# DmSM-1/C-OFDM

Hardware: AMD Instinct MI355X
Metric: IQ-samples/sec (tx IFFT+CP and rx FFT+equalise), 2048-subcarrier frames, 1/2/4/8 GPU (higher is better)
Workload: dtype f64

## Files before the change

### c-ofdm_amd/csrc/ofdm_capi.cpp

```cpp
#include <dlfcn.h>
#include <hip/hip_runtime.h>

#include <algorithm>
#include <climits>
#include <cctype>
#include <cmath>
#include <complex>
#include <cstdarg>
#include <cstdio>
#include <cstdlib>
#include <chrono>
#include <mutex>
#include <cstring>
#include <fstream>
#include <iterator>
#include <random>
#include <stdexcept>
#include <string>
#include <unordered_map>
#include <vector>

#include "../../include/ofdm_mi355x.h"

#if __has_include(<rccl/rccl.h>)
// ... 66 lines not shown
            return fail(OFDM_ERR_PARSE, "stol failed for key '%s': %s", key.c_str(), e.what());
        }
    }
    return OFDM_OK;
}

template <class T>
int upload(T** dst, const std::vector<T>& v)
{
    HIP_TRY(hipMalloc((void**)dst, std::max<size_t>(1, v.size()) * sizeof(T)));
    if (!v.empty()) HIP_TRY(hipMemcpy(*dst, v.data(), v.size() * sizeof(T), hipMemcpyHostToDevice));
    return OFDM_OK;
}

}

struct ofdm_ctx {
    ofdm_params p{};
    int device = 0;
    int logn = 0;
    int N = 0, D = 0, P = 0, cp = 0, S = 0, k = 0, L = 0, seg = 0, npr = 0, t2 = 0;
    ofdm_geometry geo{};
    std::vector<cd> t2_symbol, ofdm_preamble, mod_preamble, templ;
    std::vector<uint8_t> preamble_bytes;
    std::vector<double> t2_mask;
    double2* d_tw = nullptr;
    int* d_data_bin = nullptr;
    int* d_data_slot = nullptr;
    int* d_pilot_bin = nullptr;
    int* d_bin_map = nullptr;
    int* d_rx_pack = nullptr;
    int* d_pilot_swz = nullptr;
    int* d_tx_code = nullptr;
    double2* d_const = nullptr;
    double2* d_const_bpsk = nullptr;
    double dec_tau[3] = {};
    bool dec_fast = false;
    double2* d_header = nullptr;
    double2* d_preamble = nullptr;
    double2* d_templ = nullptr;
    double2* d_tspec = nullptr;
    float2* d_tspec32 = nullptr;
    double2* d_twm = nullptr;
    double tspec_max = 0.0;
    double2* d_modpre = nullptr;
    double* d_t2mask = nullptr;
    double2* d_t2tw = nullptr;
    int* d_first = nullptr;
    int t2_logn = -1;
    struct CfoPlan {
        int nsym = 0, logm = -1, g = 0;
        double2* tw_sub = nullptr;
        double2* tw_full = nullptr;
        int* borders = nullptr;
    };
    std::vector<CfoPlan> cfo_plans;
    double* d_cfo_scratch = nullptr;
    size_t cfo_scratch_n = 0;
    double2* d_scratch = nullptr;
    size_t scratch_bytes = 0;
    struct Grow {
        void* p = nullptr;
        size_t bytes = 0;
    };
    Grow s_walk, s_batch, s_chan, s_pbs;
    static constexpr size_t PRE_SCRATCH_STARTS = 64;
// ... 127 lines not shown
    {
        std::vector<char> used(N, 0);
        const long step = D / P + 1, seg = D / P, half = P / 2;
        long j = 0;
        auto take = [&](long b) {
            if (b < 1 || b >= N || used[b]) return false;
            used[b] = 1;
            return true;
        };
        for (long pos = 1 + seg; j < half; ++j, pos += step) {
            if (!take(pos)) return fail(OFDM_ERR_INVALID, "pilot comb does not fit fft_size");
            for (long t = 0; t < seg; ++t)
                if (!take(pos - seg + t)) return fail(OFDM_ERR_INVALID, "data segments do not fit fft_size");
        }
        for (long pos = N - step * half; j < P; ++j, pos += step) {
            if (!take(pos)) return fail(OFDM_ERR_INVALID, "pilot comb does not fit fft_size");
            for (long t = 0; t < seg; ++t)
                if (!take(pos + 1 + t)) return fail(OFDM_ERR_INVALID, "data segments do not fit fft_size");
        }
    }
    if (p->t2sin_size < 0 || (p->t2sin_size && (p->t2_sin_f1 < 0 || p->t2_sin_f1 >= p->t2sin_size ||
                                                p->t2_sin_f2 < 0 || p->t2_sin_f2 >= p->t2sin_size)))
        return fail(OFDM_ERR_INVALID, "T2 tones outside T2sin_size");
    if (p->pr_sin_len < 0 || p->pr_sin_len > (N + p->cp_size) * p->num_pr_symb)
        return fail(OFDM_ERR_INVALID, "pr_sin_len exceeds the preamble");
    return OFDM_OK;
}

int ofdm_destroy(ofdm_ctx* c)
{
    if (!c) return OFDM_OK;
    (void)hipSetDevice(c->device);
    void* ptrs[] = {c->d_tw, c->d_data_bin, c->d_data_slot, c->d_pilot_bin, c->d_bin_map, c->d_rx_pack,
                    c->d_pilot_swz, c->d_tx_code, c->d_const,
                    c->d_const_bpsk, c->d_header, c->d_preamble, c->d_templ, c->d_tspec, c->d_tspec32, c->d_twm, c->d_modpre,
                    c->d_t2mask,
                    c->d_t2tw, c->d_first, c->d_scratch, c->d_cfo_scratch, c->d_pre_hv, c->d_pre_done};
    for (void* q : ptrs)
        if (q) (void)hipFree(q);
    for (auto* g : {&c->s_walk, &c->s_batch, &c->s_chan, &c->s_pbs, &c->s_pub, &c->s_chain})
        if (g->p) (void)hipFree(g->p);
    for (auto* g : {&c->h_walk, &c->h_frames, &c->h_status})
        if (g->p) (void)hipHostFree(g->p);
    if (c->d_queue) (void)hipFree(c->d_queue);
    if (c->d_rxq) (void)hipFree(c->d_rxq);
    if (c->ev_call) (void)hipEventDestroy(c->ev_call);
    if (c->ev_walk) (void)hipEventDestroy(c->ev_walk);
    if (c->ev_wdone) (void)hipEventDestroy(c->ev_wdone);
    if (c->side) (void)hipStreamDestroy(c->side);
    for (hipEvent_t ev : c->ev_phase)
        if (ev) (void)hipEventDestroy(ev);
    for (auto& pl : c->cfo_plans) {
        if (pl.tw_sub) (void)hipFree(pl.tw_sub);
        if (pl.tw_full) (void)hipFree(pl.tw_full);
        if (pl.borders) (void)hipFree(pl.borders);
    }
    delete c;
    return OFDM_OK;
}

using ofdm::twiddles;

static std::vector<double2> constellation(int k)
{
    std::vector<double2> t(1u << k);
    if (k == 1) {
        const double step = M_PI * 2 / (double)2;
// ... 50 lines not shown

    std::vector<int> pilot(c->P), segst(c->P), data_bin(c->D), data_slot(c->D), bin_map(c->N, -1);
    {
        const int step = c->seg + 1, half = c->P / 2;
        int j = 0;
        for (int pos = 1 + c->seg; j < half; ++j, pos += step) {
            pilot[j] = pos;
            segst[j] = pos - c->seg;
        }
        for (int pos = c->N - step * half; j < c->P; ++j, pos += step) {
            pilot[j] = pos;
            segst[j] = pos + 1;
        }
        for (int jj = 0; jj < c->P; ++jj) {
            g.pilot_bin[jj] = pilot[jj];
            g.segment_bin[jj] = segst[jj];
            bin_map[pilot[jj]] = -2;
            for (int t = 0; t < c->seg; ++t) {
                const int d = jj * c->seg + t;
                data_bin[d] = segst[jj] + t;
                data_slot[d] = jj;
                bin_map[segst[jj] + t] = d;
            }
        }
    }
    std::vector<int> rx_pack(std::max(c->D, ofdm::RX_DPT * (c->N / 8)), 0),
        pilot_swz(std::max(c->P, c->N / 8), 0);
    for (int d = 0; d < c->D; ++d) rx_pack[d] = ofdm::lds_swz_host(data_bin[d]) | (data_slot[d] << 16);
    for (int j = 0; j < c->P; ++j) pilot_swz[j] = ofdm::lds_swz_host(pilot[j]);
    std::vector<int> tx_code(c->N);
    for (int b = 0; b < c->N; ++b)
        tx_code[b] = bin_map[b] >= 0 ? ofdm::tx_code_data(bin_map[b])
                                     : ofdm::tx_code_fixed(bin_map[b] == -2 ? ofdm::TX_LDS_PILOT : ofdm::TX_LDS_ZERO);
    if ((rc = upload(&c->d_rx_pack, rx_pack)) || (rc = upload(&c->d_pilot_swz, pilot_swz)) ||
        (rc = upload(&c->d_tx_code, tx_code)) ||
        (rc = upload(&c->d_tw, twiddles(c->N))) || (rc = upload(&c->d_data_bin, data_bin)) ||
        (rc = upload(&c->d_data_slot, data_slot)) || (rc = upload(&c->d_pilot_bin, pilot)) ||
        (rc = upload(&c->d_bin_map, bin_map)) || (rc = upload(&c->d_const, constellation(c->k))) ||
        (rc = upload(&c->d_const_bpsk, constellation(1)))) {
        ofdm_destroy(c);
        return rc;
    }

    if (c->k == 2) {
        double* d_tau = nullptr;
        double h_tau[4] = {};
        hipError_t e = hipMalloc((void**)&d_tau, sizeof(h_tau));
        if (e == hipSuccess) e = ofdm::launch_decide_tau_scan(c->k, d_tau, nullptr);
        if (e == hipSuccess) e = hipMemcpy(h_tau, d_tau, sizeof(h_tau), hipMemcpyDeviceToHost);
        if (d_tau) (void)hipFree(d_tau);
        if (e != hipSuccess) {
            ofdm_destroy(c);
            return hip_fail(e, "decision threshold scan");
        }
        for (int j = 0; j < 3; ++j) c->dec_tau[j] = h_tau[j];
        c->dec_fast = h_tau[3] == 1.0;
    }

    c->t2_symbol.assign(c->t2, cd(0, 0));
    if (c->t2) {
        std::vector<cd> spec(c->t2, cd(0, 0));
        spec[params->t2_sin_f1] = cd(0.5, 0);
        spec[params->t2_sin_f2] = cd(0.5, 0);
        for (int n = 0; n < c->t2; ++n) {
            cd acc(0, 0);
            for (int kk = 0; kk < c->t2; ++kk) {
// ... 201 lines not shown
    } else {
        return fail(OFDM_ERR_UNSUPPORTED, "pilot_freq_sinh: form length %ld is not 2^a or 5*2^a (64 <= 2^a <= %d)", S,
                    4096);
    }
    const int P = c->P;
    const double rel_bw = double(c->D + c->P) / (c->N);
    const double rel_pilot_w = rel_bw / P;
    const int pilot_w = int(S * rel_pilot_w);
    std::vector<int> borders(P + 2);
    for (int i = 0, j = int((1.0 - rel_bw - rel_pilot_w) / 2.0 * S); i < P + 2; i++) {
        borders[i] = j;
        j += pilot_w;
    }
    borders[0] = std::max(0, borders[0]);
    for (int b : borders)
        if (b < 0 || b > S) return fail(OFDM_ERR_UNSUPPORTED, "pilot_freq_sinh windows leave the spectrum");
    int rc;
    if ((rc = upload(&pl.tw_sub, twiddles(1 << pl.logm))) || (rc = upload(&pl.borders, borders))) return rc;
    if (pl.g == 5 && (rc = upload(&pl.tw_full, twiddles((int)S)))) return rc;
    c->cfo_plans.push_back(pl);
    *out = &c->cfo_plans.back();
    return OFDM_OK;
}

int ofdm_get_geometry(const ofdm_ctx* c, ofdm_geometry* o)
{
    if (!c || !o) return fail(OFDM_ERR_INVALID, "null argument");
    *o = c->geo;
    return OFDM_OK;
}

int ofdm_rx_emit_fast(const ofdm_ctx* c) { return c ? (c->dec_fast ? 1 : 0) : -1; }

int ofdm_get_t2_symbol(const ofdm_ctx* c, double* o)
{
    if (!c || !o) return fail(OFDM_ERR_INVALID, "null argument");
    std::memcpy(o, c->t2_symbol.data(), c->t2_symbol.size() * sizeof(cd));
    return OFDM_OK;
}

int ofdm_get_preamble(const ofdm_ctx* c, uint8_t* bytes, double* pre, double* modp, double* templ)
{
    if (!c) return fail(OFDM_ERR_INVALID, "null ctx");
    if (bytes) std::memcpy(bytes, c->preamble_bytes.data(), c->preamble_bytes.size());
    if (pre) std::memcpy(pre, c->ofdm_preamble.data(), c->ofdm_preamble.size() * sizeof(cd));
    if (modp) std::memcpy(modp, c->mod_preamble.data(), c->mod_preamble.size() * sizeof(cd));
    if (templ) std::memcpy(templ, c->templ.data(), c->templ.size() * sizeof(cd));
    return OFDM_OK;
}

int ofdm_device_alloc(ofdm_ctx* c, size_t bytes, void** d)
{
    if (!c || !d) return fail(OFDM_ERR_INVALID, "null argument");
    HIP_TRY(hipSetDevice(c->device));
    HIP_TRY(hipMalloc(d, std::max<size_t>(bytes, 1)));
    return OFDM_OK;
}
int ofdm_device_free(ofdm_ctx* c, void* d)
{
    if (!c) return fail(OFDM_ERR_INVALID, "null ctx");
    if (d) HIP_TRY(hipFree(d));
    return OFDM_OK;
}
int ofdm_memcpy_h2d(ofdm_ctx* c, void* dst, const void* src, size_t n, void* st)
{
    if (!c) return fail(OFDM_ERR_INVALID, "null ctx");
// ... 94 lines not shown
    return OFDM_OK;
}

static bool aligned16(const void* p) { return ((uintptr_t)p & 15) == 0; }

static int grow(ofdm_ctx* c, ofdm_ctx::Grow& g, size_t need)
{
    if (need <= g.bytes) return OFDM_OK;
    HIP_TRY(hipSetDevice(c->device));
    if (g.p) HIP_TRY(hipFree(g.p));
    g.p = nullptr;
    g.bytes = 0;
    HIP_TRY(hipMalloc(&g.p, need));
    g.bytes = need;
    return OFDM_OK;
}

static int grow_host(ofdm_ctx* c, ofdm_ctx::Grow& g, size_t need)
{
    if (need <= g.bytes) return OFDM_OK;
    HIP_TRY(hipSetDevice(c->device));
    if (g.p) HIP_TRY(hipHostFree(g.p));
    g.p = nullptr;
    g.bytes = 0;
    HIP_TRY(hipHostMalloc(&g.p, need, hipHostMallocDefault));
    g.bytes = need;
    return OFDM_OK;
}

static void fill_tx(const ofdm_ctx* c, ofdm::TxArgs& a, const uint8_t* bytes, size_t nframes, double* iq,
                    size_t stride, int16_t* iq16, const ofdm_channel* ch)
{
    a.tab = c->tables(false);
    a.bytes = bytes;
    a.iq = reinterpret_cast<double2*>(iq);
    a.iq16 = iq16;
    a.nframes = (long)nframes;
    a.frame_stride = (long)stride;
    a.S = c->S;
    a.D = c->D;
    a.P = c->P;
    a.cp = c->cp;
    a.k = c->k;
    a.bytes_per_frame = c->geo.bytes_per_frame;
    a.pilot_ampl = (double)c->p.pilot_ampl / 1000;
    a.inv_sqrt_n = 1.0 / std::sqrt((double)c->N);
    a.mult = (double)c->p.mult;
    if (ch && ch->noise_std > 0.0) {
        a.noise_scale = ch->noise_std * M_SQRT1_2;
        a.seed = ch->seed;
        a.sample_offset = ch->sample_offset;
    }
}

int ofdm_tx_modulate(ofdm_ctx* c, const uint8_t* bytes, size_t nframes, double* iq_out, size_t frame_stride,
                     int16_t* iq16_out, const ofdm_channel* ch, void* stream)
{
    if (!c || !bytes || !iq_out) return fail(OFDM_ERR_INVALID, "null argument");
    if (frame_stride < (size_t)c->geo.message_len) return fail(OFDM_ERR_INVALID, "frame_stride < message_len");
    if (!aligned16(iq_out)) return fail(OFDM_ERR_INVALID, "iq_out must be 16-byte aligned");
    if (nframes == 0) return OFDM_OK;
    if (nframes * (size_t)c->S > 0x7fffffffu) return fail(OFDM_ERR_INVALID, "too many symbols in one call");
    ofdm::TxArgs a{};
    fill_tx(c, a, bytes, nframes, iq_out, frame_stride, iq16_out, ch);
    hipError_t e = ofdm::launch_tx(c->logn, a, (hipStream_t)stream);
    if (e != hipSuccess) return hip_fail(e, "tx_kernel launch");
// ... 1511 lines not shown
```

### c-ofdm_amd/csrc/ofdm_fft.hpp

```cpp
#pragma once
#include <hip/hip_runtime.h>
#include <cfloat>

#ifdef OFDM_PHASE_MARKS
#define OFDM_PHASE(name) asm volatile("; OFDM_PHASE " #name)
#else
#define OFDM_PHASE(name) ((void)0)
#endif

namespace ofdm {

static __device__ int g_decode_stop = 1 << 30;
#define OFDM_STOP(PROF, k)                                                   \
    do {                                                                     \
        if constexpr (PROF) {                                                \
            if ((k) >= g_decode_stop) __builtin_amdgcn_endpgm();             \
        }                                                                    \
    } while (0)

__device__ __forceinline__ double2 cadd(double2 a, double2 b) { return make_double2(a.x + b.x, a.y + b.y); }
__device__ __forceinline__ double2 csub(double2 a, double2 b) { return make_double2(a.x - b.x, a.y - b.y); }

__device__ __forceinline__ double2 cmul(double2 a, double2 b)
{
// ... 143 lines not shown
{
    lds_tw[p.dst] = p.w;
}

template <int LOGN, int JMAX = (1 << LOGN)>
__device__ __forceinline__ double2 tw_get(const double2* __restrict__ lds_tw, int j)
{
    constexpr int NHI = TwLds<LOGN>::NHI;
    const int lo = j & 63;
    const double2 wlo = lds_tw[NHI + (lo ^ ((lo >> 4) & 3))];
    if constexpr (NHI == 1 || JMAX <= 64) return wlo;
    return cmul(lds_tw[j >> 6], wlo);
}

template <int SIGN>
__device__ __forceinline__ void dft2(double2& a, double2& b)
{
    const double2 t = a;
    a = cadd(t, b);
    b = csub(t, b);
}

template <int SIGN>
__device__ __forceinline__ void dft4(double2& a0, double2& a1, double2& a2, double2& a3)
{
    const double2 t0 = cadd(a0, a2), t1 = csub(a0, a2);
    const double2 t2 = cadd(a1, a3), t3 = mul_j<SIGN>(csub(a1, a3));
    a0 = cadd(t0, t2);
    a1 = cadd(t1, t3);
    a2 = csub(t0, t2);
    a3 = csub(t1, t3);
}

template <int SIGN>
__device__ __forceinline__ void dft8(double2& x0, double2& x1, double2& x2, double2& x3,
                                     double2& x4, double2& x5, double2& x6, double2& x7)
{
    constexpr double C = 0.70710678118654752440084436210484903928483593768847;
    dft4<SIGN>(x0, x2, x4, x6);
    dft4<SIGN>(x1, x3, x5, x7);
    const double2 o1 = make_double2((x3.x - SIGN * x3.y) * C, (x3.y + SIGN * x3.x) * C);
    const double2 o2 = mul_j<SIGN>(x5);
    const double2 o3 = make_double2(-(x7.x + SIGN * x7.y) * C, (SIGN * x7.x - x7.y) * C);
    const double2 e0 = x0, e1 = x2, e2 = x4, e3 = x6, o0 = x1;
    x0 = cadd(e0, o0);
    x4 = csub(e0, o0);
    x1 = cadd(e1, o1);
    x5 = csub(e1, o1);
    x2 = cadd(e2, o2);
    x6 = csub(e2, o2);
    x3 = cadd(e3, o3);
    x7 = csub(e3, o3);
}

template <int LOGN>
struct FftShape {
    static constexpr int N = 1 << LOGN;
    static constexpr int T = N / 8;
    static constexpr int NPASS8 = LOGN / 3;
    static constexpr int REM = LOGN % 3;
    static constexpr int PADN = N;
};

template <int LOGN, int R, int NS, int SIGN>
struct PassTw {
    double2 w[8 / R];
};

template <int LOGN, int R, int NS, int SIGN>
__device__ __forceinline__ PassTw<LOGN, R, NS, SIGN> pass_twiddles(int t, const double2* __restrict__ lds_tw)
{
    constexpr int N = 1 << LOGN, T = N / 8, B = 8 / R;
    PassTw<LOGN, R, NS, SIGN> tw;
// ... 133 lines not shown
}

template <int LOGN, int PASS, int SIGN>
__device__ __forceinline__ void fft_regs_tail(double2 (&v)[8], int t, const double2* __restrict__ lds_tw,
                                              double2* __restrict__ lds)
{
    using S = FftShape<LOGN>;
    constexpr int NPASS = S::NPASS8 + (S::REM ? 1 : 0);
    constexpr bool is8 = PASS < S::NPASS8;
    constexpr int R = is8 ? 8 : (1 << S::REM);
    constexpr int NS = 1 << (3 * PASS);
    constexpr bool LAST = PASS == NPASS - 1;
    const auto tw = pass_twiddles<LOGN, R, NS, SIGN>(t, lds_tw);
    lds_barrier();
    lds_load8<LOGN>(v, t, lds);
    if constexpr (LAST) {
        stockham_apply<LOGN, R, NS, SIGN, false>(v, t, tw, lds);
    } else {
        lds_barrier();
        stockham_apply<LOGN, R, NS, SIGN>(v, t, tw, lds);
        fft_regs_tail<LOGN, PASS + 1, SIGN>(v, t, lds_tw, lds);
    }
}

template <int LOGN, int SIGN>
__device__ __forceinline__ void fft_regs(double2 (&v)[8], int t, const double2* __restrict__ lds_tw,
                                         double2* __restrict__ lds)
{
    static_assert(LOGN >= 6 && LOGN <= 12, "N must be 64..4096");
    stockham_pass<LOGN, 8, 1, SIGN>(v, t, lds_tw, lds);
    fft_regs_tail<LOGN, 1, SIGN>(v, t, lds_tw, lds);
}

template <int LOGN, int PASS, int SIGN>
__device__ __forceinline__ void fft_regs_tail_active(double2 (&v)[8], int t, const double2* __restrict__ lds_tw,
                                                     double2* __restrict__ lds, bool active)
{
    using S = FftShape<LOGN>;
    constexpr int NPASS = S::NPASS8 + (S::REM ? 1 : 0);
    constexpr bool is8 = PASS < S::NPASS8;
    constexpr int R = is8 ? 8 : (1 << S::REM);
    constexpr int NS = 1 << (3 * PASS);
    constexpr bool LAST = PASS == NPASS - 1;
    lds_barrier();
    if (active) lds_load8<LOGN>(v, t, lds);
    if constexpr (LAST) {
        if (active) stockham_pass_regs<LOGN, R, NS, SIGN>(v, t, lds_tw, lds);
    } else {
        lds_barrier();
        if (active) stockham_pass<LOGN, R, NS, SIGN>(v, t, lds_tw, lds);
        fft_regs_tail_active<LOGN, PASS + 1, SIGN>(v, t, lds_tw, lds, active);
    }
}

template <int LOGN, int SIGN>
__device__ __forceinline__ void fft_regs_active(double2 (&v)[8], int t, const double2* __restrict__ lds_tw,
                                                double2* __restrict__ lds, bool active)
{
    static_assert(LOGN >= 9 && LOGN <= 12, "N/8 must be whole waves");
    if (active) stockham_pass<LOGN, 8, 1, SIGN>(v, t, lds_tw, lds);
    fft_regs_tail_active<LOGN, 1, SIGN>(v, t, lds_tw, lds, active);
}

__device__ __forceinline__ void wave_lds_sync()
{
    asm volatile("s_waitcnt lgkmcnt(0)" ::: "memory");
// ... 105 lines not shown
```

### c-ofdm_amd/csrc/ofdm_internal.hpp

```cpp
#pragma once
#include <hip/hip_runtime.h>
#include <cmath>
#include <cstdint>
#include <vector>

namespace ofdm {

inline std::vector<double2> twiddles(int n)
{
    std::vector<double2> w(n);
    for (int j = 0; j < n; ++j) {
        const double a = 2.0 * M_PI * (double)j / (double)n;
        w[j] = make_double2(std::cos(a), -std::sin(a));
    }
    return w;
}

struct DevTables {
    const double2* tw;
    const int* data_bin;
    const int* data_slot;
    const int* pilot_bin;
    const int* bin_map;
    const int* rx_pack;
    const int* pilot_swz;
    const int* tx_code;
    const double2* constell;
};

struct TxArgs {
    DevTables tab;
    const uint8_t* bytes;
    const double2* points;
    double2* iq;
    int16_t* iq16;
    const double2* header;
    long nframes;
    long frame_stride;
    long msg_offset;
    int header_len;
    int S, D, P, cp, k;
    long bytes_per_frame;
    double pilot_ampl;
    double inv_sqrt_n;
    double mult;
    double noise_scale;
    unsigned long long seed;
    unsigned long long sample_offset;
};

constexpr int CORR_BITS = 9;
constexpr int CORR_PER_SYM = CORR_BITS + 2;

struct RxArgs {
    DevTables tab;
    const double2* iq;
    const short2* iq16;
    long nframes;
    long frame_stride;
    const double2* chan;
    long chan_stride;
    bool chan_recip;
    double2* constell;
    double2* read_out;
    uint8_t* bytes;
    const uint8_t* ref;
    unsigned long long* bit_errors;
    double2* ystage;
    const long* starts;
    long start_off;
    const long* count;
    int* queue;
    const double2* corr;
    int S, D, P, seg, cp, k;
    long bytes_per_frame;
    double pilot_ampl;
    double dec_tau[3];
    int dec_fast;
};

struct SoftArgs {
    void* llr;
    const double* frame_scale;
    double scale;
    int fmt;
};

hipError_t launch_rx_soft(int logn, const RxArgs& a, const SoftArgs& sa, hipStream_t stream);
hipError_t launch_soft_demap(const double2* pts, long n, int k, double scale, int fmt, void* out, hipStream_t stream);
hipError_t launch_tx(int logn, const TxArgs& a, hipStream_t stream);
hipError_t launch_rx(int logn, const RxArgs& a, hipStream_t stream, bool* staged_needed);
hipError_t launch_decide_tau_scan(int k, double* out, hipStream_t stream);
hipError_t launch_copy(void* dst, const void* src, size_t n, hipStream_t stream);
hipError_t launch_demap(double2* pts, long n, int k, uint8_t* bytes, hipStream_t stream);
hipError_t launch_map(const uint8_t* bytes, long nbytes, int k, const double2* table, double2* out,
                      hipStream_t stream);
hipError_t launch_bit_convert(const uint8_t* in, long len, int in_bits, int out_bits, uint8_t* out, long out_len,
                              hipStream_t stream);
hipError_t launch_i16_to_f64(const int16_t* in, long n, double* out, hipStream_t stream);
hipError_t launch_f64_to_i16(const double* in, long n, double mult, int16_t* out, hipStream_t stream);

constexpr int RX_SMAX = 8;
inline int lds_swz_host(int e) { return e ^ ((e >> 3) & 7); }
constexpr int RX_DPT = 4;
constexpr int RX_WAVES_PER_CU = 8;
constexpr int TX_LDS_PILOT = 256, TX_LDS_ZERO = 257;
inline int tx_code_data(int d) { return d | (0xff << 13); }
inline int tx_code_fixed(int entry) { return entry << 21; }
constexpr long TX_MAX_GRID = 4096;


struct FecRate { int period, kept; unsigned mask; };
__host__ __device__ inline FecRate fec_rate(int rate)
{
    return rate == 0 ? FecRate{1, 1, 0x1u} : rate == 1 ? FecRate{4, 3, 0x7u} : FecRate{6, 4, 0x27u};
}
constexpr int FEC_TAIL = 6;
constexpr long FEC_MAX_INFO_BITS = 1L << 20;
constexpr int FEC_CW_PER_WG = 4;
constexpr long FEC_LDS_STEPS = 1024;
inline long fec_steps_padded(long info_bits) { return (info_bits + FEC_TAIL + 63) & ~63L; }

struct FecEncArgs {
    const uint8_t* info;
    uint8_t* coded;
    long info_stride, coded_stride;
    long ncw, info_bits, coded_bits;
    int rate;
};

struct FecDecArgs {
    const void* llr;
    long llr_stride;
    long ncw, info_bits;
    unsigned long long* ws;
    uint8_t* out;
    const uint8_t* ref;
    unsigned long long* bit_errors;
    long info_stride;
    int fmt, rate;
    int gather;
// ... 32 lines not shown
```

### c-ofdm_amd/csrc/ofdm_kernels.hip

```cpp
#include <hip/hip_runtime.h>
#include <algorithm>
#include <cstdint>
#include <cstdlib>

#include "ofdm_dev.hpp"
#include "ofdm_fft.hpp"
#include "ofdm_internal.hpp"
#include "ofdm_rx2.hpp"

#include <type_traits>

namespace ofdm {


__device__ __forceinline__ int symbol_bits(const uint8_t* __restrict__ b, long nbytes, long g, int k)
{
    const long bit = g * k;
    const long byte = bit >> 3;
    const int off = (int)(bit & 7);
    const int mask = (1 << k) - 1;
    if (off + k <= 8) return (b[byte] >> (8 - off - k)) & mask;
    const int w = ((int)b[byte] << 8) | (byte + 1 < nbytes ? (int)b[byte + 1] : 0);
    return (w >> (16 - off - k)) & mask;
}
// ... 131 lines not shown
        if (lane == 0) r[w] = v;
        __syncthreads();
        unsigned long long s = 0;
        for (int i = 0; i < NW; ++i) s += r[i];
        return s;
    }
}

constexpr int tx_min_blocks(int logn, bool i16) { return logn == 11 && !i16 ? 4 : 1; }

template <int LOGN, bool POINTS, bool NOISE, bool I16>
__global__ void __launch_bounds__((1 << LOGN) / 8, tx_min_blocks(LOGN, I16)) tx_kernel(TxArgs a)
{
    using FS = FftShape<LOGN>;
    constexpr int N = FS::N, T = FS::T;
    extern __shared__ double2 smem[];
    double2* fft = smem;
    double2* lds_tw = smem + FS::PADN;
    double2* lds_const = lds_tw + TwLds<LOGN>::SIZE;
    uint8_t* sbytes = reinterpret_cast<uint8_t*>(lds_const + TX_LDS_ZERO + 1);
    const int t = threadIdx.x;
    load_twiddles<LOGN>(a.tab.tw, lds_tw, t, T);
    for (int i = t; i < (1 << a.k); i += T) lds_const[i] = a.tab.constell[i];
    if (t == 0) {
        lds_const[TX_LDS_PILOT] = make_double2(a.pilot_ampl, 0.0);
        lds_const[TX_LDS_ZERO] = make_double2(0.0, 0.0);
    }


    const long nsym = a.nframes * a.S;
    const int k = a.k;
    const int bps = a.D * k / 8;
    const int L = N + a.cp;
    auto sym_bytes = [&](long sym) {
        const long f = sym / a.S;
        return a.bytes + f * a.bytes_per_frame + (sym - f * a.S) * bps;
    };
    const bool by_word = (bps & 3) == 0 && (a.bytes_per_frame & 3) == 0 && ((uintptr_t)a.bytes & 3) == 0;
    const int nwords = bps >> 2;
    uint32_t nb[8];
    auto fetch = [&](long s) {
        const uint8_t* src = sym_bytes(s);
        if (by_word) {
            int tt;
            asm volatile("v_mov_b32 %0, %1" : "=v"(tt) : "v"(t));
            const int wi0 = tt < nwords ? tt : 0, wi1 = tt + T < nwords ? tt + T : 0;
            const uint32_t* w = reinterpret_cast<const uint32_t*>(src);
            nb[0] = w[wi0];
            nb[1] = w[wi1];
        } else {
#pragma unroll
            for (int r = 0; r < 8; ++r) nb[r] = src[t + T * r < bps ? t + T * r : 0];
        }
    };
    auto publish = [&]() {
        if (by_word) {
            uint32_t* w = reinterpret_cast<uint32_t*>(sbytes);
            w[t] = nb[0];
            w[t + T] = nb[1];
        } else {
#pragma unroll
            for (int r = 0; r < 8; ++r) sbytes[t + T * r] = (uint8_t)nb[r];
        }
    };

    long sym = blockIdx.x;
    if (!POINTS && sym < nsym) {
        fetch(sym);
        publish();
    }
    lds_barrier();

    const bool cp_reg = (a.cp % T) == 0;
    const int i_cp = 8 - a.cp / T;
    const int kmask = (1 << k) - 1;

    const long gstep_f = gridDim.x / a.S;
    const int gstep_s = (int)(gridDim.x - gstep_f * a.S);
    long f = sym / a.S;
    int s = (int)(sym - f * a.S);
    for (; sym < nsym; sym += gridDim.x) {
        double2 v[8];
        int code[8];
        {
            int tt;
            asm volatile("v_mov_b32 %0, %1" : "=v"(tt) : "v"(t));
            const int* ct = a.tab.tx_code + tt;
#pragma unroll
            for (int i = 0; i < 8; ++i) code[i] = ct[T * i];
        }
#pragma unroll
        for (int i = 0; i < 8; ++i) {
            const int d = code[i] & 0x1fff, m = (code[i] >> 13) & 0xff, base = code[i] >> 21;
            if constexpr (POINTS) {
                v[i] = m ? a.points[sym * a.D + d] : lds_const[base];
            } else {
                const int bit = d * k;
                const int byte = bit >> 3, off = bit & 7;
                const int w = ((int)sbytes[byte] << 8) | (int)sbytes[byte + 1];
                v[i] = lds_const[((w >> (16 - off - k)) & kmask & m) + base];
            }
        }
        const long nxt = sym + gridDim.x;
        if constexpr (!POINTS) fetch(nxt < nsym ? nxt : sym);

        fft_regs<LOGN, +1>(v, t, lds_tw, fft);
        if constexpr (!POINTS) publish();

        const long base = f * a.frame_stride + a.msg_offset + (long)s * L;
        double2* out = a.iq + base;
        int16_t* out16 = I16 ? a.iq16 + 2 * base : nullptr;
        const unsigned long long g0 = a.sample_offset + (unsigned long long)sym * L;
        const AwgnRun run = NOISE ? awgn_run(awgn_key(a.seed), g0) : AwgnRun{};
        auto emit = [&](int j, double2 z) {
            if constexpr (NOISE && !I16) {
                const double2 w = awgn_sample_scaled(run, (uint32_t)j, (float)a.noise_scale);
                store_nt(out + j, make_double2(fma(z.x, a.inv_sqrt_n, w.x), fma(z.y, a.inv_sqrt_n, w.y)));
                return;
            }
            z.x *= a.inv_sqrt_n;
            z.y *= a.inv_sqrt_n;
            if constexpr (I16) {
                const uint32_t w = (uint16_t)to_int16(z.x * a.mult) | ((uint32_t)(uint16_t)to_int16(z.y * a.mult) << 16);
                __builtin_nontemporal_store(w, reinterpret_cast<uint32_t*>(out16 + 2 * j));
            }
            if constexpr (NOISE) {
                const double2 w = awgn_sample(run, (uint32_t)j, a.noise_scale);
                z.x += w.x;
                z.y += w.y;
            }
            store_nt(out + j, z);
        };
        if (cp_reg) {
#pragma unroll
            for (int i = 0; i < 8; ++i)
                if (i >= i_cp) emit(t + T * i - (N - a.cp), v[i]);
        } else {
            int tt;
            asm volatile("v_mov_b32 %0, %1" : "=v"(tt) : "v"(t));
            lds_barrier();
#pragma unroll
            for (int i = 0; i < 8; ++i)
                if (tt + T * i >= N - a.cp) fft[lds_swz(tt + T * i)] = v[i];
            lds_barrier();
            for (int j = tt; j < a.cp; j += T) emit(j, fft[lds_swz(N - a.cp + j)]);
        }
#pragma unroll
        for (int i = 0; i < 8; ++i) emit(a.cp + t + T * i, v[i]);
        if (a.header && s == 0) {
            double2* fr = a.iq + f * a.frame_stride;
            int16_t* fr16 = I16 ? a.iq16 + 2 * f * a.frame_stride : nullptr;
            for (int j = t; j < a.header_len; j += T) {
                const double2 z = a.header[j];
                fr[j] = z;
                if constexpr (I16) {
                    fr16[2 * j] = to_int16(z.x * a.mult);
                    fr16[2 * j + 1] = to_int16(z.y * a.mult);
                }
            }
        }
        lds_barrier();
        s += gstep_s;
        f += gstep_f;
        if (s >= a.S) {
            s -= a.S;
            ++f;
        }
    }
}

template <int LOGN, bool I16>
struct SymbolRegs;

template <int LOGN>
struct SymbolRegs<LOGN, false> {
    double2 r[8];
    __device__ __forceinline__ void load(const RxArgs& a, long off, int t)
    {
        constexpr int T = (1 << LOGN) / 8;
#pragma unroll
        for (int i = 0; i < 8; ++i)
            r[i] = load_nt(a.iq + off + t + T * i);
    }
    __device__ __forceinline__ double2 get(int i) const { return r[i]; }
};

template <int LOGN>
struct SymbolRegs<LOGN, true> {
    int r[8];
    __device__ __forceinline__ void load(const RxArgs& a, long off, int t)
    {
        constexpr int T = (1 << LOGN) / 8;
        const int* p = reinterpret_cast<const int*>(a.iq16 + off);
#pragma unroll
        for (int i = 0; i < 8; ++i) r[i] = __builtin_nontemporal_load(p + t + T * i);
    }
    __device__ __forceinline__ double2 get(int i) const
    {
        return make_double2((double)(int)(short)(r[i] & 0xffff), (double)(r[i] >> 16));
    }
// ... 639 lines not shown
```

### c-ofdm_amd/python/ofdm_mi355x.py

```python
from __future__ import annotations

import ctypes as C
import os
import subprocess

HERE = os.path.dirname(os.path.abspath(__file__))
PKG = os.path.dirname(HERE)
LIB_PATH = os.environ.get("OFDM_MI355X_LIB") or os.path.join(PKG, "lib", "libofdm_mi355x.so")
HEADER = os.path.join(os.path.dirname(PKG), "include", "ofdm_mi355x.h")

PARAM_FIELDS = [
    "fft_size", "num_data_subc", "num_pilot_subc", "cp_size", "num_symb", "num_pr_symb",
    "pr_sin_len", "pr_seed", "pr_level", "t2sin_size", "t2_sin_f1", "t2_sin_f2",
    "t2_sin_level", "smooth", "mod_type", "pilot_ampl", "mult", "rx_buf_size", "iterations",
]

OFDM_OK = 0
ERRORS = {-1: "INVALID", -2: "UNSUPPORTED", -3: "HIP", -4: "IO", -5: "NOMEM", -6: "PARSE"}
LLR_F32, LLR_I8 = 0, 1
FEC_R12, FEC_R23, FEC_R34 = 0, 1, 2
IL_FORWARD, IL_INVERSE = 0, 1
SYNC_CFO, SYNC_FREQ_SHIFT, SYNC_CP, SYNC_PHASE, SYNC_CHAN, SYNC_ALL = 1, 2, 4, 8, 16, 31


# ... 21 lines not shown
class Channel(C.Structure):
    _fields_ = [("noise_std", C.c_double), ("seed", C.c_ulonglong), ("sample_offset", C.c_ulonglong)]


class WalkTuning(C.Structure):
    _fields_ = [("chunks_per_slot", C.c_long), ("halo_milli", C.c_long), ("ext_milli", C.c_long),
                ("exact_search", C.c_int), ("t2_f32", C.c_int), ("t2_margin", C.c_double),
                ("allow_uncertified", C.c_int), ("staged_decode", C.c_int), ("lookback", C.c_int),
                ("max_rec_cap", C.c_int), ("pre_f32", C.c_int)]


class WalkState(C.Structure):
    _fields_ = [("pos", C.c_long), ("ring_end", C.c_long)]


class OfdmError(RuntimeError):
    def __init__(self, code: int, msg: str):
        super().__init__(f"ofdm error {code} ({ERRORS.get(code, '?')}): {msg}")
        self.code = code


_V, _I, _L, _SZ, _D = C.c_void_p, C.c_int, C.c_long, C.c_size_t, C.c_double
_PP = C.POINTER(Params)
SIGNATURES = {
    "ofdm_last_error": (C.c_char_p, []),
    "ofdm_abi_version": (_I, []),
    "ofdm_params_default": (_I, [_PP]),
    "ofdm_params_from_config": (_I, [C.c_char_p, _PP]),
    "ofdm_config_lookup": (_I, [C.c_char_p, C.c_char_p, C.POINTER(C.c_long)]),
    "ofdm_create": (_I, [_PP, _I, C.POINTER(_V)]),
    "ofdm_destroy": (_I, [_V]),
    "ofdm_get_geometry": (_I, [_V, C.POINTER(Geometry)]),
    "ofdm_rx_emit_fast": (_I, [_V]),
    "ofdm_get_t2_symbol": (_I, [_V, _V]),
    "ofdm_get_preamble": (_I, [_V, _V, _V, _V, _V]),
    "ofdm_device_alloc": (_I, [_V, _SZ, C.POINTER(_V)]),
    "ofdm_device_free": (_I, [_V, _V]),
    "ofdm_memcpy_h2d": (_I, [_V, _V, _V, _SZ, _V]),
    "ofdm_memcpy_d2h": (_I, [_V, _V, _V, _SZ, _V]),
    "ofdm_copy": (_I, [_V, _V, _V, _SZ, _V]),
    "ofdm_rx_demod_read": (_I, [_V, _V, _SZ, _SZ, _V, _SZ, _V, _V, _V, _V]),
    "ofdm_memset_device": (_I, [_V, _V, _I, _SZ, _V]),
    "ofdm_stream_synchronize": (_I, [_V, _V]),
    "ofdm_tx_modulate": (_I, [_V, _V, _SZ, _V, _SZ, _V, C.POINTER(Channel), _V]),
    "ofdm_tx_frames": (_I, [_V, _V, _SZ, _V, _V, _V]),
    "ofdm_rx_demod": (_I, [_V, _V, _SZ, _SZ, _V, _SZ, _V, _V, _V, _V, _V]),
    "ofdm_rx_demod_i16": (_I, [_V, _V, _SZ, _SZ, _V, _SZ, _V, _V, _V, _V, _V]),
    "ofdm_demap": (_I, [_V, _V, _SZ, _V, _V]),
    "ofdm_soft_demap": (_I, [_V, _V, _SZ, _D, _I, _V, _V]),
    "ofdm_rx_demod_soft": (_I, [_V, _V, _V, _SZ, _SZ, _V, _SZ, _D, _V, _I, _V, _V, _V, _V, _V, _V]),
    "ofdm_chan_estimate_ls": (_I, [_V, _V, _SZ, _SZ, _I, _V, _SZ, _V, _SZ, _V]),
    "ofdm_soft_demap_csi": (_I, [_V, _V, _SZ, _V, _SZ, _D, _V, _I, _V, _V]),
    "ofdm_fec_coded_bits": (_I, [_SZ, _I, C.POINTER(_SZ)]),
    "ofdm_fec_max_info_bits": (_I, [_SZ, _I, C.POINTER(_SZ)]),
    "ofdm_fec_workspace_size": (_I, [_SZ, _SZ, C.POINTER(_SZ)]),
    "ofdm_fec_encode": (_I, [_V, _V, _SZ, _SZ, _SZ, _I, _V, _SZ, _V]),
    "ofdm_fec_decode": (_I, [_V, _V, _I, _SZ, _SZ, _SZ, _I, _V, _SZ, _V, _SZ, _V, _V, _V]),
    "ofdm_interleave_default": (_I, [_V, C.POINTER(_SZ), C.POINTER(_SZ), C.POINTER(_SZ)]),
    "ofdm_interleave_bits": (_I, [_V, _V, _SZ, _SZ, _SZ, _SZ, _I, _V, _V]),
    "ofdm_interleave_llr": (_I, [_V, _V, _I, _SZ, _SZ, _SZ, _SZ, _I, _V, _V]),
    "ofdm_scramble": (_I, [_V, _V, _SZ, _SZ, _SZ, C.c_uint, _V, _V, _SZ, _V]),
    "ofdm_map": (_I, [_V, _V, _SZ, _V, _V]),
    "ofdm_fft_write": (_I, [_V, _V, _SZ, _V, _V]),
    "ofdm_fft_read": (_I, [_V, _V, _SZ, _V, _V]),
    "ofdm_bit_convert": (_I, [_V, _V, _SZ, _I, _I, _V, C.POINTER(_SZ), _V]),
    "ofdm_int16_to_double": (_I, [_V, _V, _SZ, _V, _V]),
# ... 116 lines not shown
        import torch
        return torch.cuda.current_stream().cuda_stream
    return stream if isinstance(stream, int) else stream.cuda_stream


class Modem:

    def __init__(self, params, device: int = 0):
        if isinstance(params, dict):
            params = Params.make(**params)
        self.params = params
        self.device = device
        h = C.c_void_p()
        check(lib().ofdm_create(C.byref(params), device, C.byref(h)))
        self.h = h
        g = Geometry()
        check(lib().ofdm_get_geometry(h, C.byref(g)))
        self.geo = g

    def close(self):
        if getattr(self, "h", None):
            lib().ofdm_destroy(self.h)
            self.h = None

    def __del__(self):
        try:
            self.close()
        except Exception:
            pass

    def rx_emit_fast(self) -> bool:
        return lib().ofdm_rx_emit_fast(self.h) == 1

    def t2_symbol(self):
        import numpy as np
        out = np.zeros(self.params.t2sin_size, np.complex128)
        check(lib().ofdm_get_t2_symbol(self.h, out.ctypes.data))
        return out

    def preamble(self):
        import numpy as np
        p = self.params
        b = np.zeros(p.num_data_subc * p.num_pr_symb // 8, np.uint8)
        pre = np.zeros(self.geo.preamble_len, np.complex128)
        modp = np.zeros(p.num_data_subc * p.num_pr_symb, np.complex128)
        tpl = np.zeros(p.pr_sin_len, np.complex128)
        check(lib().ofdm_get_preamble(self.h, b.ctypes.data, pre.ctypes.data, modp.ctypes.data,
                                      tpl.ctypes.data))
        return b, pre, modp, tpl

    def tx(self, data, nframes: int, iq_out, frame_stride: int | None = None, iq16_out=None,
           noise_std: float = 0.0, seed: int = 0, sample_offset: int = 0, stream=None):
        stride = self.geo.message_len if frame_stride is None else frame_stride
        ch = Channel(noise_std, seed, sample_offset) if noise_std > 0 else None
        check(lib().ofdm_tx_modulate(self.h, _ptr(data), nframes, _ptr(iq_out), stride,
                                     _ptr(iq16_out), C.byref(ch) if ch else None, _stream(stream)))

    def tx_frames(self, data, nframes: int, frames_out, frames16_out=None, stream=None):
        check(lib().ofdm_tx_frames(self.h, _ptr(data), nframes, _ptr(frames_out), _ptr(frames16_out),
                                   _stream(stream)))

    def rx(self, iq, nframes: int, frame_stride: int | None = None, chan=None, chan_stride: int = 0,
           constell_out=None, bytes_out=None, ref=None, bit_errors=None, stream=None):
        stride = self.geo.message_len if frame_stride is None else frame_stride
        check(lib().ofdm_rx_demod(self.h, _ptr(iq), nframes, stride, _ptr(chan), chan_stride,
                                  _ptr(constell_out), _ptr(bytes_out), _ptr(ref), _ptr(bit_errors),
# ... 227 lines not shown
```

### include/ofdm_mi355x.h

```cpp
#ifndef OFDM_MI355X_H
#define OFDM_MI355X_H

#include <stddef.h>
#include <stdint.h>

#ifdef __cplusplus
extern "C" {
#endif

#define OFDM_MI355X_ABI_VERSION 5

enum {
    OFDM_OK = 0,
    OFDM_ERR_INVALID = -1,
    OFDM_ERR_UNSUPPORTED = -2,
    OFDM_ERR_HIP = -3,
    OFDM_ERR_IO = -4,
    OFDM_ERR_NOMEM = -5,
    OFDM_ERR_PARSE = -6
};

typedef struct ofdm_params {
    long fft_size;
    long num_data_subc;
// ... 18 lines not shown

typedef struct ofdm_geometry {
    long symbol_len;
    long message_len;
    long preamble_len;
    long frame_len;
    long ring_len;
    long data_per_frame;
    long bytes_per_frame;
    long segment_size;
    long pilot_bin[256];
    long segment_bin[256];
} ofdm_geometry;

typedef struct ofdm_channel {
    double noise_std;
    unsigned long long seed;
    unsigned long long sample_offset;
} ofdm_channel;

typedef struct ofdm_ctx ofdm_ctx;

const char* ofdm_last_error(void);
int ofdm_abi_version(void);

int ofdm_params_default(ofdm_params* out);
int ofdm_params_from_config(const char* path, ofdm_params* out);
int ofdm_config_lookup(const char* path, const char* key, long* value);

int ofdm_create(const ofdm_params* params, int device, ofdm_ctx** out);
int ofdm_destroy(ofdm_ctx* ctx);
int ofdm_get_geometry(const ofdm_ctx* ctx, ofdm_geometry* out);
int ofdm_rx_emit_fast(const ofdm_ctx* ctx);
int ofdm_get_t2_symbol(const ofdm_ctx* ctx, double* out );
int ofdm_get_preamble(const ofdm_ctx* ctx,
                      uint8_t* bytes_out ,
                      double* ofdm_preamble_out ,
                      double* mod_preamble_out ,
                      double* template_out );

int ofdm_device_alloc(ofdm_ctx* ctx, size_t bytes, void** dptr);
int ofdm_device_free(ofdm_ctx* ctx, void* dptr);
int ofdm_memcpy_h2d(ofdm_ctx* ctx, void* dst, const void* src, size_t bytes, void* stream);
int ofdm_memcpy_d2h(ofdm_ctx* ctx, void* dst, const void* src, size_t bytes, void* stream);
int ofdm_memset_device(ofdm_ctx* ctx, void* dst, int value, size_t bytes, void* stream);
int ofdm_stream_synchronize(ofdm_ctx* ctx, void* stream);
int ofdm_host_alloc(ofdm_ctx* ctx, size_t bytes, void** hptr);
int ofdm_host_free(ofdm_ctx* ctx, void* hptr);
int ofdm_stream_create(ofdm_ctx* ctx, void** stream);
int ofdm_stream_destroy(ofdm_ctx* ctx, void* stream);
int ofdm_memcpy_d2d(ofdm_ctx* ctx, void* dst, const void* src, size_t bytes, void* stream);
int ofdm_copy(ofdm_ctx* ctx, void* dst, const void* src, size_t bytes, void* stream);
int ofdm_event_create(ofdm_ctx* ctx, void** event);
int ofdm_event_record(ofdm_ctx* ctx, void* event, void* stream);
int ofdm_event_synchronize(ofdm_ctx* ctx, void* event);
int ofdm_event_destroy(ofdm_ctx* ctx, void* event);

int ofdm_tx_modulate(ofdm_ctx* ctx, const uint8_t* bytes, size_t nframes,
                     double* iq_out, size_t frame_stride, int16_t* iq16_out,
                     const ofdm_channel* ch, void* stream);

int ofdm_tx_frames(ofdm_ctx* ctx, const uint8_t* bytes, size_t nframes,
                   double* frames_out, int16_t* frames16_out, void* stream);

int ofdm_rx_demod(ofdm_ctx* ctx, const double* iq, size_t nframes, size_t frame_stride,
                  const double* chan, size_t chan_stride,
// ... 178 lines not shown
```

Baseline: 143.8 billion.

## Prune first IFFT radix-8 stage for wavefronts whose input bins are all zero

Precomputes per-wavefront masks marking which of the eight register slots map only to zero (guard/DC) subcarriers, uploads them, and in the tx kernel dispatches to a pruned radix-8 first pass that skips code-table loads, constellation lookups and butterfly arithmetic for those known-zero inputs. It also restructures the frame/symbol index stepping so the next symbol's byte address is computed once and reused for prefetch. This adds template instantiations (three first-pass variants), which may raise code size and register pressure, and a new API toggle for the sparse path.

```diff
diff --git a/c-ofdm_amd/csrc/ofdm_capi.cpp b/c-ofdm_amd/csrc/ofdm_capi.cpp
--- a/c-ofdm_amd/csrc/ofdm_capi.cpp
+++ b/c-ofdm_amd/csrc/ofdm_capi.cpp
@@ -122,6 +122,13 @@
     int* d_rx_pack = nullptr;
     int* d_pilot_swz = nullptr;
     int* d_tx_code = nullptr;
+    std::vector<int> tx_code;
+    std::vector<unsigned> tx_dead;
+    unsigned* d_tx_dead = nullptr;
+#ifndef OFDM_TX_SPARSE_DEFAULT
+#define OFDM_TX_SPARSE_DEFAULT 1
+#endif
+    bool tx_sparse = OFDM_TX_SPARSE_DEFAULT != 0;
     double2* d_const = nullptr;
     double2* d_const_bpsk = nullptr;
     double dec_tau[3] = {};
@@ -315,7 +322,7 @@
     if (!c) return OFDM_OK;
     (void)hipSetDevice(c->device);
     void* ptrs[] = {c->d_tw, c->d_data_bin, c->d_data_slot, c->d_pilot_bin, c->d_bin_map, c->d_rx_pack,
-                    c->d_pilot_swz, c->d_tx_code, c->d_const,
+                    c->d_pilot_swz, c->d_tx_code, c->d_tx_dead, c->d_const,
                     c->d_const_bpsk, c->d_header, c->d_preamble, c->d_templ, c->d_tspec, c->d_tspec32, c->d_twm, c->d_modpre,
                     c->d_t2mask,
                     c->d_t2tw, c->d_first, c->d_scratch, c->d_cfo_scratch, c->d_pre_hv, c->d_pre_done};
@@ -432,6 +439,13 @@
     for (int b = 0; b < c->N; ++b)
         tx_code[b] = bin_map[b] >= 0 ? ofdm::tx_code_data(bin_map[b])
                                      : ofdm::tx_code_fixed(bin_map[b] == -2 ? ofdm::TX_LDS_PILOT : ofdm::TX_LDS_ZERO);
+    c->tx_code = tx_code;
+    c->tx_dead = ofdm::tx_dead_masks(tx_code);
+    if (std::any_of(c->tx_dead.begin(), c->tx_dead.end(), [](unsigned m) { return m != 0; }) &&
+        (rc = upload(&c->d_tx_dead, c->tx_dead))) {
+        ofdm_destroy(c);
+        return rc;
+    }
     if ((rc = upload(&c->d_rx_pack, rx_pack)) || (rc = upload(&c->d_pilot_swz, pilot_swz)) ||
         (rc = upload(&c->d_tx_code, tx_code)) ||
         (rc = upload(&c->d_tw, twiddles(c->N))) || (rc = upload(&c->d_data_bin, data_bin)) ||
@@ -699,6 +713,15 @@
 
 int ofdm_rx_emit_fast(const ofdm_ctx* c) { return c ? (c->dec_fast ? 1 : 0) : -1; }
 
+int ofdm_tx_sparse(ofdm_ctx* c, int enable, unsigned* masks_out, int* codes_out)
+{
+    if (!c) return -1;
+    if (enable >= 0) c->tx_sparse = enable != 0;
+    if (masks_out) std::copy(c->tx_dead.begin(), c->tx_dead.end(), masks_out);
+    if (codes_out) std::copy(c->tx_code.begin(), c->tx_code.end(), codes_out);
+    return c->tx_sparse && c->d_tx_dead ? 1 : 0;
+}
+
 int ofdm_get_t2_symbol(const ofdm_ctx* c, double* o)
 {
     if (!c || !o) return fail(OFDM_ERR_INVALID, "null argument");
@@ -859,6 +882,7 @@
                     size_t stride, int16_t* iq16, const ofdm_channel* ch)
 {
     a.tab = c->tables(false);
+    a.tx_dead = c->tx_sparse ? c->d_tx_dead : nullptr;
     a.bytes = bytes;
     a.iq = reinterpret_cast<double2*>(iq);
     a.iq16 = iq16;
diff --git a/c-ofdm_amd/csrc/ofdm_fft.hpp b/c-ofdm_amd/csrc/ofdm_fft.hpp
--- a/c-ofdm_amd/csrc/ofdm_fft.hpp
+++ b/c-ofdm_amd/csrc/ofdm_fft.hpp
@@ -199,13 +199,45 @@
     a3 = csub(t1, t3);
 }
 
-template <int SIGN>
+template <int SIGN, bool Z1, bool Z2>
+__device__ __forceinline__ void dft4z(double2& a0, double2& a1, double2& a2, double2& a3)
+{
+    const double2 t0 = Z2 ? a0 : cadd(a0, a2), t1 = Z2 ? a0 : csub(a0, a2);
+    if constexpr (Z1) {
+        const double2 t2 = a3, j3 = mul_j<SIGN>(a3);
+        a0 = cadd(t0, t2);
+        a1 = csub(t1, j3);
+        a2 = csub(t0, t2);
+        a3 = cadd(t1, j3);
+    } else {
+        const double2 t2 = cadd(a1, a3), t3 = mul_j<SIGN>(csub(a1, a3));
+        a0 = cadd(t0, t2);
+        a1 = cadd(t1, t3);
+        a2 = csub(t0, t2);
+        a3 = csub(t1, t3);
+    }
+}
+
+enum Dft8Zeros {
+    DFT8_FULL = 0,
+    DFT8_Z2345 = 0x3c,
+    DFT8_Z34 = 0x18,
+};
+
+template <int SIGN, int ZEROS = DFT8_FULL>
 __device__ __forceinline__ void dft8(double2& x0, double2& x1, double2& x2, double2& x3,
                                      double2& x4, double2& x5, double2& x6, double2& x7)
 {
+    static_assert(ZEROS == DFT8_FULL || ZEROS == DFT8_Z2345 || ZEROS == DFT8_Z34, "no pruned form for this pattern");
     constexpr double C = 0.70710678118654752440084436210484903928483593768847;
-    dft4<SIGN>(x0, x2, x4, x6);
-    dft4<SIGN>(x1, x3, x5, x7);
+    constexpr bool z2 = (ZEROS >> 2) & 1, z3 = (ZEROS >> 3) & 1, z4 = (ZEROS >> 4) & 1, z5 = (ZEROS >> 5) & 1;
+    if constexpr (ZEROS == DFT8_FULL) {
+        dft4<SIGN>(x0, x2, x4, x6);
+        dft4<SIGN>(x1, x3, x5, x7);
+    } else {
+        dft4z<SIGN, z2, z4>(x0, x2, x4, x6);
+        dft4z<SIGN, z3, z5>(x1, x3, x5, x7);
+    }
     const double2 o1 = make_double2((x3.x - SIGN * x3.y) * C, (x3.y + SIGN * x3.x) * C);
     const double2 o2 = mul_j<SIGN>(x5);
     const double2 o3 = make_double2(-(x7.x + SIGN * x7.y) * C, (SIGN * x7.x - x7.y) * C);
@@ -405,6 +437,15 @@
     fft_regs_tail<LOGN, 1, SIGN>(v, t, lds_tw, lds);
 }
 
+template <int LOGN, int SIGN, int ZEROS>
+__device__ __forceinline__ void fft_regs_first(double2 (&v)[8], int t, double2* __restrict__ lds)
+{
+    static_assert(LOGN >= 6 && LOGN <= 12, "N must be 64..4096");
+    dft8<SIGN, ZEROS>(v[0], v[1], v[2], v[3], v[4], v[5], v[6], v[7]);
+#pragma unroll
+    for (int r = 0; r < 8; ++r) lds[lds_swz(8 * t + r)] = v[r];
+}
+
 template <int LOGN, int PASS, int SIGN>
 __device__ __forceinline__ void fft_regs_tail_active(double2 (&v)[8], int t, const double2* __restrict__ lds_tw,
                                                      double2* __restrict__ lds, bool active)
diff --git a/c-ofdm_amd/csrc/ofdm_internal.hpp b/c-ofdm_amd/csrc/ofdm_internal.hpp
--- a/c-ofdm_amd/csrc/ofdm_internal.hpp
+++ b/c-ofdm_amd/csrc/ofdm_internal.hpp
@@ -47,6 +47,7 @@
     double noise_scale;
     unsigned long long seed;
     unsigned long long sample_offset;
+    const unsigned* tx_dead;
 };
 
 constexpr int CORR_BITS = 9;
@@ -107,6 +108,18 @@
 constexpr int TX_LDS_PILOT = 256, TX_LDS_ZERO = 257;
 inline int tx_code_data(int d) { return d | (0xff << 13); }
 inline int tx_code_fixed(int entry) { return entry << 21; }
+inline std::vector<unsigned> tx_dead_masks(const std::vector<int>& tx_code)
+{
+    const int T = (int)tx_code.size() / 8;
+    std::vector<unsigned> m(T / 64, 0u);
+    for (int w = 0; w < T / 64; ++w)
+        for (int i = 0; i < 8; ++i) {
+            bool dead = true;
+            for (int lane = 0; lane < 64; ++lane) dead = dead && tx_code[64 * w + lane + T * i] == tx_code_fixed(TX_LDS_ZERO);
+            if (dead) m[w] |= 1u << i;
+        }
+    return m;
+}
 constexpr long TX_MAX_GRID = 4096;
 
 
diff --git a/c-ofdm_amd/csrc/ofdm_kernels.hip b/c-ofdm_amd/csrc/ofdm_kernels.hip
--- a/c-ofdm_amd/csrc/ofdm_kernels.hip
+++ b/c-ofdm_amd/csrc/ofdm_kernels.hip
@@ -187,15 +187,11 @@
     const int k = a.k;
     const int bps = a.D * k / 8;
     const int L = N + a.cp;
-    auto sym_bytes = [&](long sym) {
-        const long f = sym / a.S;
-        return a.bytes + f * a.bytes_per_frame + (sym - f * a.S) * bps;
-    };
+    auto sym_bytes = [&](long f, int s) { return a.bytes + f * a.bytes_per_frame + (long)s * bps; };
     const bool by_word = (bps & 3) == 0 && (a.bytes_per_frame & 3) == 0 && ((uintptr_t)a.bytes & 3) == 0;
     const int nwords = bps >> 2;
     uint32_t nb[8];
-    auto fetch = [&](long s) {
-        const uint8_t* src = sym_bytes(s);
+    auto fetch = [&](const uint8_t* src) {
         if (by_word) {
             int tt;
             asm volatile("v_mov_b32 %0, %1" : "=v"(tt) : "v"(t));
@@ -220,46 +216,78 @@
     };
 
     long sym = blockIdx.x;
-    if (!POINTS && sym < nsym) {
-        fetch(sym);
-        publish();
-    }
-    lds_barrier();
-
-    const bool cp_reg = (a.cp % T) == 0;
-    const int i_cp = 8 - a.cp / T;
-    const int kmask = (1 << k) - 1;
-
     const long gstep_f = gridDim.x / a.S;
     const int gstep_s = (int)(gridDim.x - gstep_f * a.S);
     long f = sym / a.S;
     int s = (int)(sym - f * a.S);
+    if (!POINTS && sym < nsym) {
+        fetch(sym_bytes(f, s));
+        publish();
+    }
+    lds_barrier();
+
+    const bool cp_reg = (a.cp % T) == 0;
+    const int i_cp = 8 - a.cp / T;
+    const int kmask = (1 << k) - 1;
+
+    unsigned dead = 0;
+    if constexpr (T >= 64) {
+        if (a.tx_dead) dead = __builtin_amdgcn_readfirstlane(a.tx_dead[t >> 6]);
+    }
+
     for (; sym < nsym; sym += gridDim.x) {
+        long fn = f + gstep_f;
+        int sn = s + gstep_s;
+        if (sn >= a.S) {
+            sn -= a.S;
+            ++fn;
+        }
+        const bool more = sym + gridDim.x < nsym;
         double2 v[8];
-        int code[8];
-        {
-            int tt;
-            asm volatile("v_mov_b32 %0, %1" : "=v"(tt) : "v"(t));
-            const int* ct = a.tab.tx_code + tt;
-#pragma unroll
-            for (int i = 0; i < 8; ++i) code[i] = ct[T * i];
-        }
-#pragma unroll
-        for (int i = 0; i < 8; ++i) {
-            const int d = code[i] & 0x1fff, m = (code[i] >> 13) & 0xff, base = code[i] >> 21;
-            if constexpr (POINTS) {
-                v[i] = m ? a.points[sym * a.D + d] : lds_const[base];
-            } else {
-                const int bit = d * k;
-                const int byte = bit >> 3, off = bit & 7;
-                const int w = ((int)sbytes[byte] << 8) | (int)sbytes[byte + 1];
-                v[i] = lds_const[((w >> (16 - off - k)) & kmask & m) + base];
+        auto map_first = [&](auto zeros) {
+            constexpr int ZEROS = decltype(zeros)::value;
+            int code[8];
+            {
+                int tt;
+                asm volatile("v_mov_b32 %0, %1" : "=v"(tt) : "v"(t));
+                const int* ct = a.tab.tx_code + tt;
+#pragma unroll
+                for (int i = 0; i < 8; ++i)
+                    if (!((ZEROS >> i) & 1)) code[i] = ct[T * i];
             }
-        }
-        const long nxt = sym + gridDim.x;
-        if constexpr (!POINTS) fetch(nxt < nsym ? nxt : sym);
-
-        fft_regs<LOGN, +1>(v, t, lds_tw, fft);
+#pragma unroll
+            for (int i = 0; i < 8; ++i) {
+                if ((ZEROS >> i) & 1) {
+                    v[i] = make_double2(0.0, 0.0);
+                    continue;
+                }
+                const int d = code[i] & 0x1fff, m = (code[i] >> 13) & 0xff, base = code[i] >> 21;
+                if constexpr (POINTS) {
+                    v[i] = m ? a.points[sym * a.D + d] : lds_const[base];
+                } else {
+                    const int bit = (int)__umul24((unsigned)d, (unsigned)k);
+                    const int byte = bit >> 3, off = bit & 7;
+                    const int w = ((int)sbytes[byte] << 8) | (int)sbytes[byte + 1];
+                    v[i] = lds_const[((w >> (16 - off - k)) & kmask & m) + base];
+                }
+            }
+            if constexpr (!POINTS) fetch(more ? sym_bytes(fn, sn) : sym_bytes(f, s));
+            if constexpr (ZEROS == DFT8_FULL)
+                stockham_pass<LOGN, 8, 1, +1>(v, t, lds_tw, fft);
+            else
+                fft_regs_first<LOGN, +1, ZEROS>(v, t, fft);
+        };
+        if constexpr (T >= 64) {
+            if ((dead & DFT8_Z2345) == DFT8_Z2345)
+                map_first(std::integral_constant<int, DFT8_Z2345>());
+            else if ((dead & DFT8_Z34) == DFT8_Z34)
+                map_first(std::integral_constant<int, DFT8_Z34>());
+            else
+                map_first(std::integral_constant<int, DFT8_FULL>());
+        } else {
+            map_first(std::integral_constant<int, DFT8_FULL>());
+        }
+        fft_regs_tail<LOGN, 1, +1>(v, t, lds_tw, fft);
         if constexpr (!POINTS) publish();
 
         const long base = f * a.frame_stride + a.msg_offset + (long)s * L;
@@ -315,12 +343,8 @@
             }
         }
         lds_barrier();
-        s += gstep_s;
-        f += gstep_f;
-        if (s >= a.S) {
-            s -= a.S;
-            ++f;
-        }
+        f = fn;
+        s = sn;
     }
 }
 
diff --git a/c-ofdm_amd/python/ofdm_mi355x.py b/c-ofdm_amd/python/ofdm_mi355x.py
--- a/c-ofdm_amd/python/ofdm_mi355x.py
+++ b/c-ofdm_amd/python/ofdm_mi355x.py
@@ -77,6 +77,7 @@
     "ofdm_destroy": (_I, [_V]),
     "ofdm_get_geometry": (_I, [_V, C.POINTER(Geometry)]),
     "ofdm_rx_emit_fast": (_I, [_V]),
+    "ofdm_tx_sparse": (_I, [_V, _I, _V, _V]),
     "ofdm_get_t2_symbol": (_I, [_V, _V]),
     "ofdm_get_preamble": (_I, [_V, _V, _V, _V, _V]),
     "ofdm_device_alloc": (_I, [_V, _SZ, C.POINTER(_V)]),
@@ -259,6 +260,16 @@
     def rx_emit_fast(self) -> bool:
         return lib().ofdm_rx_emit_fast(self.h) == 1
 
+    def tx_sparse(self, enable: bool | None = None) -> bool:
+        return lib().ofdm_tx_sparse(self.h, -1 if enable is None else int(enable), None, None) == 1
+
+    def tx_dead_tables(self):
+        import numpy as np
+        n = self.params.fft_size
+        masks, codes = np.zeros(n // 512, np.uint32), np.zeros(n, np.int32)
+        lib().ofdm_tx_sparse(self.h, -1, masks.ctypes.data, codes.ctypes.data)
+        return masks, codes
+
     def t2_symbol(self):
         import numpy as np
         out = np.zeros(self.params.t2sin_size, np.complex128)
diff --git a/include/ofdm_mi355x.h b/include/ofdm_mi355x.h
--- a/include/ofdm_mi355x.h
+++ b/include/ofdm_mi355x.h
@@ -74,6 +74,7 @@
 int ofdm_destroy(ofdm_ctx* ctx);
 int ofdm_get_geometry(const ofdm_ctx* ctx, ofdm_geometry* out);
 int ofdm_rx_emit_fast(const ofdm_ctx* ctx);
+int ofdm_tx_sparse(ofdm_ctx* ctx, int enable, unsigned* masks_out, int* codes_out);
 int ofdm_get_t2_symbol(const ofdm_ctx* ctx, double* out );
 int ofdm_get_preamble(const ofdm_ctx* ctx,
                       uint8_t* bytes_out ,
```

New measurement: 146.8 billion (median of 6 runs). 2.1% higher.
